# ferreiraluisa/implementation-phd-lab-vision

Measured on AMD Instinct MI355X. Metric: H36M frames/sec ResNet-50 feature extraction, higher is better.
Workload: dtype bf16; 1 GPU; ResNet-50[:-1] bf16 forward, batch 256 x 224x224x3 fp32 NCHW frames per GPU (BASELINE configs[1]), seeded synthetic weights, (N,2048) fp32 features; batch_per_gpu=256, micro_batch=0, lanes=2, lanes_requested=2, lanes_mode=2 lanes (1.081 x one lane), input=f32, parallelism=frames sharded over 1 rank(s)

## Files before the change

### implementation_phd_lab_vision_amd/_lib.py

```python
from __future__ import annotations

import ctypes as C
import os
import subprocess
from pathlib import Path
from typing import Optional

PKG_DIR = Path(__file__).resolve().parent
LIB_PATH = Path(os.environ.get("R50_LIB", str(PKG_DIR / "libr50hip.so")))
CSRC = PKG_DIR / "csrc"

HIPCC_FLAGS = ["--offload-arch=gfx950", "-O3", "-std=c++17", "-fPIC", "-shared", "-ffp-contract=off"]


class R50Error(RuntimeError):
    pass


class TensorDesc(C.Structure):
    _fields_ = [("name", C.c_char_p), ("data", C.POINTER(C.c_float)), ("numel", C.c_int64)]


def _source_digest() -> str:
    import hashlib
# ... 82 lines not shown
                                            C.c_void_p, C.c_int, C.c_void_p]),
    "r50_op_transpose16": (C.c_int, [C.c_void_p, C.c_int, C.c_int, C.c_void_p, C.c_int, C.c_void_p]),
    "r50_op_mask_scale": (C.c_int, [C.c_void_p, C.c_void_p, C.c_float, C.c_int64, C.c_int, C.c_void_p]),
    "r50_op_relu_bwd": (C.c_int, [C.c_void_p, C.c_void_p, C.c_float, C.c_int64, C.c_int, C.c_void_p]),
    "r50_op_colsum": (C.c_int, [C.c_void_p, C.c_int64, C.c_int, C.c_int, C.c_float, C.c_void_p, C.c_int, C.c_int, C.c_void_p]),
    "r50_op_colsum_f32": (C.c_int, [C.c_void_p, C.c_int64, C.c_int, C.c_float, C.c_void_p, C.c_int, C.c_void_p]),
    "r50_op_grad_accum": (C.c_int, [C.c_void_p, C.c_float, C.c_void_p, C.c_int64, C.c_int, C.c_int, C.c_void_p]),
    "r50_op_mse_loss_grad": (C.c_int, [C.c_void_p, C.c_void_p, C.c_int64, C.c_float, C.c_void_p, C.c_void_p, C.c_void_p]),
    "r50_op_gn_relu_causal3_bwd": (C.c_int, [C.c_void_p, C.c_void_p, C.c_int, C.c_int, C.c_int, C.c_int, C.c_void_p, C.c_void_p,
                                             C.c_float, C.c_void_p, C.c_void_p, C.c_void_p, C.c_void_p, C.c_int, C.c_void_p]),
    "r50_op_check_finite": (C.c_int, [C.c_void_p, C.c_int64, C.c_void_p, C.c_void_p]),
    "r50_op_check_overflow16": (C.c_int, [C.c_void_p, C.c_int64, C.c_void_p, C.c_int, C.c_void_p]),
    "r50_op_adamw": (C.c_int, [C.c_void_p, C.c_void_p, C.c_void_p, C.c_void_p, C.c_void_p, C.c_int64, C.c_float, C.c_float, C.c_float,
                               C.c_float, C.c_float, C.c_int, C.c_void_p, C.c_int, C.c_void_p]),
    "r50_op_avgpool": (C.c_int, [C.c_void_p, C.c_int, C.c_int, C.c_int, C.c_void_p, C.c_void_p]),
    "r50_op_pose_metrics": (C.c_int, [C.c_void_p, C.c_void_p, C.c_int64, C.c_int, C.c_void_p, C.c_void_p]),
    "r50_op_horizon_metrics": (C.c_int, [C.c_void_p, C.c_void_p, C.c_int, C.c_int, C.c_int, C.c_int, C.c_int, C.c_void_p, C.c_void_p]),
    "r50_op_pose_protocols": (C.c_int, [C.c_void_p, C.c_void_p, C.c_void_p, C.c_int, C.c_int, C.c_int, C.c_int, C.c_int, C.c_int,
                                        C.c_int, C.c_void_p, C.c_void_p]),
    "r50_op_pose_detail_metrics": (C.c_int, [C.c_void_p, C.c_void_p, C.c_void_p, C.c_int, C.c_int, C.c_int, C.c_int, C.c_int, C.c_int,
                                             C.c_int, C.c_int, C.c_double, C.c_void_p, C.c_void_p]),
    "r50_op_future_pose_loss_grad": (C.c_int, [C.c_void_p, C.c_void_p, C.c_int, C.c_int, C.c_int, C.c_float, C.c_void_p, C.c_void_p,
                                               C.c_void_p]),
    "r50_op_ar_latent_grad": (C.c_int, [C.c_void_p, C.c_void_p, C.c_void_p, C.c_int, C.c_int, C.c_int, C.c_float, C.c_float, C.c_void_p,
                                        C.c_void_p, C.c_void_p, C.c_int, C.c_void_p]),
    "r50_op_colsum_split": (C.c_int, [C.c_void_p, C.c_int64, C.c_int, C.c_int, C.c_float, C.c_void_p, C.c_void_p, C.c_int, C.c_int,
                                      C.c_void_p]),
    "r50_op_joint_pose_loss_grad": (C.c_int, [C.c_void_p, C.c_void_p, C.c_int, C.c_int, C.c_int, C.c_float, C.c_float, C.c_void_p,
                                              C.c_void_p, C.c_void_p]),
    "r50_op_gn_relu_causal3_tm_bwd": (C.c_int, [C.c_void_p, C.c_void_p, C.c_int, C.c_int, C.c_int, C.c_int, C.c_int, C.c_void_p, C.c_void_p,
# ... 38 lines not shown
```

### implementation_phd_lab_vision_amd/csrc/kernels.h

```cpp
#pragma once
#include <hip/hip_runtime.h>
#include <stdint.h>
#include <type_traits>

typedef __attribute__((ext_vector_type(8))) __bf16 bf16x8;
typedef __attribute__((ext_vector_type(4))) float f32x4;
typedef __attribute__((ext_vector_type(4))) unsigned int u32x4;
typedef __attribute__((ext_vector_type(2))) unsigned int u32x2;

#define GLOBAL_AS __attribute__((address_space(1)))
#define LDS_AS __attribute__((address_space(3)))

__device__ __forceinline__ float bf16_bits_to_f32(unsigned int hi16) { return __uint_as_float(hi16 << 16); }

__device__ __forceinline__ unsigned int pack_bf16x2(float lo, float hi) {
    typedef __attribute__((ext_vector_type(2))) __bf16 bf16x2;
    typedef __attribute__((ext_vector_type(2))) float f32x2;
    f32x2 v = {lo, hi};
    bf16x2 b = __builtin_convertvector(v, bf16x2);
    return __builtin_bit_cast(unsigned int, b);
}

typedef __attribute__((ext_vector_type(8))) _Float16 f16x8;
typedef __attribute__((ext_vector_type(2))) _Float16 f16x2;
// ... 67 lines not shown
    int n_blocks;
    int x_back;
    unsigned x_records;
    unsigned w_bytes;
    unsigned y_bytes;
    FastDiv div_howo, div_wo, div_ctiles;
    int x_cstride;
    int x_wrap;
    int y_cstride;
    int et;
    float oscale, rscale;
    float q_inv;
    const __bf16* x2;
    int H2, W2, stride2, x2_cstride, cc1;
    unsigned x2_records;
#if defined(R50_STAMP)
    unsigned long long* dbg;
#endif
};

#if defined(R50_STAMP)
#define R50_STAMP_DECL unsigned long long st_prev = __builtin_readcyclecounter(), st_sum[8] = {0, 0, 0, 0, 0, 0, 0, 0}; const unsigned long long st_rt0 = __builtin_amdgcn_s_memrealtime();
#define R50_MARK(i) { __builtin_amdgcn_sched_barrier(0); const unsigned long long st_now = __builtin_readcyclecounter(); st_sum[i] += st_now - st_prev; st_prev = st_now; __builtin_amdgcn_sched_barrier(0); }
#define R50_STAMP_FLUSH(nw) st_sum[7] = __builtin_amdgcn_s_memrealtime() - st_rt0;    \
    if (a.dbg && (threadIdx.x & 63) == 0) { _Pragma("unroll") for (int q = 0; q < 8; ++q) \
        a.dbg[((size_t)blockIdx.x * (nw) + (threadIdx.x >> 6)) * 8 + q] = st_sum[q]; }
#else
#define R50_STAMP_DECL
#define R50_MARK(i)
#define R50_STAMP_FLUSH(nw)
// ... 20 lines not shown
        constexpr int MID = (LO + HI) / 2;
        if (n <= MID) wait_vmcnt_range<LO, MID>(n);
        else wait_vmcnt_range<MID + 1, HI>(n);
    }
}
__device__ __forceinline__ void wait_vmcnt(int n) { wait_vmcnt_range<0, 63>(n < 0 ? 0 : (n > 63 ? 63 : n)); }

__device__ __forceinline__ unsigned relu_bf16x2(unsigned v) {
    typedef __attribute__((ext_vector_type(2))) short s16x2;
    const s16x2 z = {0, 0};
    return __builtin_bit_cast(unsigned, __builtin_elementwise_max(__builtin_bit_cast(s16x2, v), z));
}

constexpr unsigned kOobOffset = 0x80000000u;

template <int ET, int BC, int BP, int WC, int WP, int NSTAGE, bool SPLIT = false>
__global__ __launch_bounds__(WC * WP * 64) void igemm_bf16_kernel(const ConvArgs a) {
#if defined(__HIP_DEVICE_COMPILE__)
    constexpr int NT = WC * WP * 64;
    constexpr int MR = BC / WC / 16;
    constexpr int NR = BP / WP / 16;
    static_assert(MR >= 2 && (MR % 2) == 0, "wave needs >= 32 couts");
    static_assert(NSTAGE == 2 || NSTAGE == 3, "2 or 3 LDS stages");
    constexpr int RPP = NT / 8;
    static_assert(BC % RPP == 0 && BP % (16 * WP) == 0, "cout rows fill whole staging passes; pixels come in 16-blocks per wave");
    constexpr int WROWS = BC / RPP;
    constexpr int XROWS = (BP + RPP - 1) / RPP;
    constexpr int BP_PAD = XROWS * RPP;
    constexpr int PASS_BYTES = NT * 16;
    constexpr int STAGE_BYTES = (BC + BP_PAD) * 128;
    constexpr int LOADS_PER_STAGE = WROWS + XROWS;
    constexpr int D = NSTAGE - 1;

    extern __shared__ __attribute__((aligned(16))) char smem[];

    const int tid = threadIdx.x;
    const int lane = tid & 63;
    const int wave = __builtin_amdgcn_readfirstlane(tid >> 6);
    const int wave_c = wave / WP, wave_p = wave % WP;
    const int fr = lane & 15, fq = lane >> 4;
    const int srow = tid >> 3;
    const int slot = tid & 7;
    const int lchunk = slot ^ (srow & 7);

    const int grid = gridDim.x;
    const int first = xcd_remap(blockIdx.x, grid);
    const int my_tiles = (a.n_blocks - first + grid - 1) / grid;
    const int total = my_tiles * a.nk;

    const __amdgpu_buffer_rsrc_t rsrc_w =
        __builtin_amdgcn_make_buffer_rsrc(const_cast<__bf16*>(a.w), 0, a.w_bytes, 0x00020000);
    const __amdgpu_buffer_rsrc_t rsrc_x = __builtin_amdgcn_make_buffer_rsrc(
        const_cast<char*>(reinterpret_cast<const char*>(a.x) - a.x_back), 0, a.x_records, 0x00020000);
    const __amdgpu_buffer_rsrc_t rsrc_y = __builtin_amdgcn_make_buffer_rsrc(a.y, 0, a.y_bytes, 0x00020000);
    const __amdgpu_buffer_rsrc_t rsrc_r =
        __builtin_amdgcn_make_buffer_rsrc(const_cast<__bf16*>(a.res), 0, a.res ? a.y_bytes : 0u, 0x00020000);

    unsigned x_voff[XROWS], x_mask[XROWS], w_voff[WROWS];
    auto decode_tile = [&](int tile) {
        const int pt = (int)fast_div((unsigned)tile, a.div_ctiles);
        const int ct = tile - pt * a.n_ctiles;
        const int c0 = ct * BC, p0 = pt * BP;
#pragma unroll
        for (int i = 0; i < XROWS; ++i) {
            const int m = p0 + i * RPP + srow;
            unsigned mask = 0u, voff = kOobOffset;
            if ((BP_PAD == BP || i * RPP + srow < BP) && m < a.M) {
                const int n = (int)fast_div((unsigned)m, a.div_howo);
                const int r = m - n * a.HoWo;
                const int ho = (int)fast_div((unsigned)r, a.div_wo);
                const int wo = r - ho * a.Wo;
                const int hc = ho * a.stride, wc = wo * a.stride;
                voff = (unsigned)(((n * a.H + hc) * a.W + wc) * a.x_cstride + lchunk * 8) * 2u;
                if (a.ks == 1) {
                    mask = 1u;
                } else {
                    const unsigned hm = (hc >= a.pad ? 1u : 0u) | 2u | (hc - a.pad + 2 < a.H ? 4u : 0u);
                    const unsigned wm = (wc >= a.pad ? 1u : 0u) | 2u | (wc - a.pad + 2 < a.W ? 4u : 0u);
                    mask = ((hm & 1u) ? wm : 0u) | ((hm & 2u) ? (wm << 3) : 0u) | ((hm & 4u) ? (wm << 6) : 0u);
                }
            }
            x_voff[i] = voff;
// ... 40 lines not shown
        }
    };

    f32x4 acc[MR][NR];
    constexpr bool BIG = (MR * NR > 16);
    constexpr bool LEAN = (NT >= 1024);
    constexpr bool PREFETCH_RES = !SPLIT && !BIG && !LEAN;
    u32x4 res_reg[PREFETCH_RES ? MR / 2 : 1][PREFETCH_RES ? NR : 1];
    const bool has_res = (a.res != nullptr);
    const int fphys0 = (fq ^ (fr & 7)) << 4;
    const int w_frag = (wave_c * MR * 16 + fr) * 128;
    const int x_frag = BC * 128 + (wave_p * NR * 16 + fr) * 128;
    const int cout_lane = wave_c * MR * 16 + 8 * fq;
    const int pix_lane = wave_p * NR * 16 + fr;
    int c_tile = first, c_k = 0, c_buf = 0;
    unsigned y_voff = 0u;
    const unsigned y_rowstep = (unsigned)(16 * a.y_cstride * 2);

    auto tile_begin = [&]() {
        const int pt = (int)fast_div((unsigned)c_tile, a.div_ctiles);
        const int c0 = (c_tile - pt * a.n_ctiles) * BC, p0 = pt * BP;
        y_voff = (unsigned)((p0 + pix_lane) * a.y_cstride + c0 + cout_lane) * 2u;
#pragma unroll
        for (int t = 0; t < MR / 2; ++t) {
            const f32x4 b_lo = *reinterpret_cast<const f32x4*>(a.bias + c0 + cout_lane + 32 * t);
            const f32x4 b_hi = *reinterpret_cast<const f32x4*>(a.bias + c0 + cout_lane + 32 * t + 4);
#pragma unroll
            for (int j = 0; j < NR; ++j) {
                acc[2 * t][j] = b_lo;
                acc[2 * t + 1][j] = b_hi;
                if constexpr (PREFETCH_RES) if (has_res)
                    res_reg[t][j] = __builtin_amdgcn_raw_buffer_load_b128(rsrc_r, y_voff + j * y_rowstep + 64 * t, 0, 0);
            }
        }
    };
    auto compute = [&]() {
        const char* sbase = smem + c_buf * STAGE_BYTES;
// ... 25 lines not shown
                wf[kk][m] = *reinterpret_cast<const bf16x8*>(sbase + w_frag + m * 2048 + ph);
        }
#pragma unroll
        for (int kk = 0; kk < 2; ++kk)
#pragma unroll
            for (int m = 0; m < MR; ++m)
#pragma unroll
                for (int j = 0; j < NR; ++j)
                    acc[m][j] = mfma_e<ET>(wf[kk][m], xf[kk][j], acc[m][j]);
        if constexpr (BIG) {
            __builtin_amdgcn_sched_group_barrier(0x100, 2 * (MR + NR), 0);
            __builtin_amdgcn_sched_group_barrier(0x008, 2 * MR * NR, 0);
        }
        }
    };
    auto epilogue = [&]() {
#pragma unroll
        for (int t = 0; t < MR / 2; ++t) {
#pragma unroll
            for (int j = 0; j < NR; ++j) {
                f32x4 lo = acc[2 * t][j], hi = acc[2 * t + 1][j];
                const unsigned voff = y_voff + j * y_rowstep + 64 * t;
                if constexpr (!SPLIT) {
                    if (has_res) {
                        u32x4 r;
                        if constexpr (PREFETCH_RES) r = res_reg[t][j];
                        else r = __builtin_amdgcn_raw_buffer_load_b128(rsrc_r, voff, 0, 0);
                        lo[0] += unpack_lo_e<ET>(r[0]); lo[1] += unpack_hi_e<ET>(r[0]);
                        lo[2] += unpack_lo_e<ET>(r[1]); lo[3] += unpack_hi_e<ET>(r[1]);
                        hi[0] += unpack_lo_e<ET>(r[2]); hi[1] += unpack_hi_e<ET>(r[2]);
                        hi[2] += unpack_lo_e<ET>(r[3]); hi[3] += unpack_hi_e<ET>(r[3]);
// ... 32 lines not shown
                }
            }
        }
    };

#pragma unroll
    for (int s = 0; s < D; ++s)
        if (s < total) stage_issue();
    for (int g = 0; g < total; ++g) {
        if (NSTAGE == 3 && g + 1 < total) {
            asm volatile("s_waitcnt vmcnt(%0)" ::"n"(LOADS_PER_STAGE) : "memory");
        } else {
            asm volatile("s_waitcnt vmcnt(0)" ::: "memory");
        }
        __builtin_amdgcn_s_barrier();
        if (c_k == 0) tile_begin();
        if (g + D < total) stage_issue();
        compute();
        c_buf = (c_buf == NSTAGE - 1) ? 0 : c_buf + 1;
        if (++c_k == a.nk) {
            epilogue();
            c_k = 0;
            c_tile += grid;
        }
    }
#else
    (void)a;
#endif
}

template <int ET, int BC, int BP, int CWC, int CWP, int NLOAD, int NSTAGE>
__global__ __launch_bounds__((CWC * CWP + NLOAD) * 64) void igemm_ws_kernel(const ConvArgs a) {
#if defined(__HIP_DEVICE_COMPILE__)
    constexpr int NCONS = CWC * CWP;
    constexpr int MR = BC / CWC / 16;
    constexpr int NR = BP / CWP / 16;
    static_assert(MR >= 2 && (MR % 2) == 0, "consumer wave needs >= 32 couts");
    static_assert(BP % (16 * CWP) == 0, "pixels come in 16-blocks per consumer wave");
// ... 4795 lines not shown
```

### implementation_phd_lab_vision_amd/csrc/r50_abi.hip

```cpp
#include "kernels.h"
#include "../../include/r50.h"

#include <atomic>
#include <cmath>
#include <cstdlib>
#include <cstdio>
#include <cstring>
#include <map>
#include <string>
#include <vector>

namespace {

thread_local std::string g_err;

struct Prof {
    const char* name;
    int64_t launches = 0;
    double ms = 0, flops = 0, bytes = 0;
};
enum ProfClass { PC_IGEMM = 0, PC_STEM_CONV, PC_MAXPOOL, PC_AVGPOOL, PC_STEM_PACK, PC_TAIL, PC_TAIL3, PC_BLOCK2, PC_CATCHAIN, PC_COUNT };
const char* kProfNames[PC_COUNT] = {"igemm", "conv1", "maxpool", "avgpool", "stem_pack", "bneck_tail", "bneck_tail3", "bneck_block2", "bneck_catchain"};

struct EvRec {
// ... 31 lines not shown
    std::vector<float> fp8_scales;
    float cat_acc_scale[4] = {0.f, 0.f, 0.f, 0.f};
    int fuse_ds_cat = 1;
    __bf16* cat_w[4] = {nullptr, nullptr, nullptr, nullptr};
    float* cat_bias[4] = {nullptr, nullptr, nullptr, nullptr};
    int fuse_tail = 1;
    int fuse_fp8_handover = 1;
    int fuse_tail3 = 1;
    __bf16* catchain_wp = nullptr;
    int fuse_tail3_last = 1;
    int fuse_cat_chain = 1;
    int sub_out = 1;
    __bf16* tail3_wp[8] = {nullptr, nullptr, nullptr, nullptr, nullptr, nullptr, nullptr, nullptr};
    int fuse_block1 = 3;
    int fuse_block2 = 1;
    int inplace_out = 0;
    int n_streams = 1;
    hipStream_t side[4] = {nullptr, nullptr, nullptr, nullptr};
    hipEvent_t ev_fork = nullptr, ev_join[4] = {nullptr, nullptr, nullptr, nullptr};
    bool loaded = false;
    r50_handle* owner = nullptr;
    int sharers = 0;
    bool zombie = false;
    std::string err;
    std::vector<ConvLayer> convs;
    char* stem_w = nullptr;
    char* stem_xp = nullptr;
    float* u8_table = nullptr;
    __bf16* buf[5] = {nullptr, nullptr, nullptr, nullptr, nullptr};
    size_t buf_bytes = 0;
// ... 217 lines not shown
            int dev = 0;
            hipDeviceProp_t prop;
            if (hipGetDevice(&dev) != hipSuccess || hipGetDeviceProperties(&prop, dev) != hipSuccess) return hipErrorInvalidDevice;
            g_num_cus = cu_budget(prop.multiProcessorCount);
        }
        static int per_cu = 0;
        if (per_cu == 0) {
            int n = 0;
            if (hipOccupancyMaxActiveBlocksPerMultiprocessor(&n, kern, WC * WP * 64, lds) != hipSuccess || n < 1) n = 1;
            per_cu = n;
        }
        if (grid > g_num_cus * per_cu) grid = g_num_cus * per_cu;
    }
    hipLaunchKernelGGL(kern, dim3(grid), dim3(WC * WP * 64), lds, s, a);
    return hipGetLastError();
}

struct TunedTile { int h, cin, cout, ks, stride, res, tile; };
constexpr TunedTile kTuned[] = {
    {56, 64, 64, 1, 1, 0, 73},    {56, 64, 64, 3, 1, 0, 2},     {56, 64, 256, 1, 1, 1, 72},   {56, 64, 256, 1, 1, 0, 38},
    {56, 256, 64, 1, 1, 0, 73},    {56, 256, 128, 1, 1, 0, 40},  {56, 128, 128, 3, 2, 0, 65},   {28, 128, 512, 1, 1, 1, 72},
    {56, 256, 512, 1, 2, 0, 42},  {28, 512, 128, 1, 1, 0, 65},   {28, 128, 128, 3, 1, 0, 72},  {28, 512, 256, 1, 1, 0, 72},
    {28, 256, 256, 3, 2, 0, 44},  {14, 256, 1024, 1, 1, 1, 72}, {28, 512, 1024, 1, 2, 0, 72}, {14, 1024, 256, 1, 1, 0, 44},
    {14, 256, 256, 3, 1, 0, 68},  {14, 1024, 512, 1, 1, 0, 72}, {14, 512, 512, 3, 2, 0, 68},  {7, 512, 2048, 1, 1, 1, 43},
    {14, 1024, 2048, 1, 2, 0, 43}, {7, 2048, 512, 1, 1, 0, 72}, {7, 512, 512, 3, 1, 0, 68},
};

constexpr int kWsBit = 64;

template <int ET, int BC, int BP, int CWC, int CWP, int NLOAD, int NSTAGE>
// ... 282 lines not shown
    a.cin_chunks = kmul * (cin / 64); a.nk = ks * ks * a.cin_chunks; a.Ktot = ks * ks * kmul * cin;
    a.n_ctiles = 0; a.n_blocks = 0;
    const long long x_bytes = (long long)n * h * w * a.x_cstride * 2;
    a.x_back = (pad * w + pad) * a.x_cstride * 2;
    if (x_bytes + a.x_back >= (1ll << 31) || (long long)cout * a.Ktot * 2 >= (1ll << 31) || M * a.y_cstride * 2 >= (1ll << 31))
        return R50_ERR_INVALID;
    a.x_records = (unsigned)(x_bytes + a.x_back);
    a.w_bytes = (unsigned)((long long)cout * a.Ktot * 2);
    a.y_bytes = (unsigned)(M * a.y_cstride * 2);
    a.div_howo = make_fast_div((unsigned)a.HoWo);
    a.div_wo = make_fast_div((unsigned)a.Wo);
    a.div_ctiles = FastDiv{0u, 0u};
    a.et = 0;
    a.oscale = 1.0f; a.rscale = 1.0f; a.q_inv = 0.0f;
    a.x2 = nullptr; a.H2 = 0; a.W2 = 0; a.stride2 = 1; a.x2_cstride = 0; a.cc1 = 1 << 30; a.x2_records = 0u;
#if defined(R50_STAMP)
    a.dbg = nullptr;
#endif
    return R50_OK;
}

void prof_begin(r50_handle* h, hipStream_t s, EvRec& r, int cls, double flops, double bytes, int layer = -1) {
    if (!h || !h->profile) return;
    r.layer = layer;
    auto get = [&]() {
        hipEvent_t e;
        if (!h->ev_free.empty()) { e = h->ev_free.back(); h->ev_free.pop_back(); }
        else (void)hipEventCreate(&e);
        return e;
    };
// ... 510 lines not shown
    }
    if (hit("stem", buf[0], 112, 112, 64)) return R50_OK;

    prof_begin(h, s, r, PC_MAXPOOL, 0, (double)n * (112.0 * 112 + 56.0 * 56) * 64 * 2 * cmul);
    e = split ? launch_maxpool_split(buf[0], buf[1], n, 112, 112, 64, s) : launch_maxpool(buf[0], buf[1], n, 112, 112, 64, s, et);
    prof_end(h, s, r);
    if (e != hipSuccess) return fail(h, R50_ERR_HIP, std::string("maxpool: ") + hipGetErrorString(e));
after_pool:
    if (hit("pool", buf[1], 56, 56, 64)) return R50_OK;

    int cur = 1, hh = 56, ww = 56;
    int pre_t1 = stem_c1 ? 2 : -1;
    bool layer1_out_fp8 = false;
    bool cur_sub = false;
    size_t li = 1;
    for (int si = 0; si < 4; ++si) {
        const int blocks = kStages[si][1];
        if (si == 1 && h->precision == R50_PREC_FP8) {
            if (tap) return fail(h, R50_ERR_INVALID, "fp8 mode: activations beyond layer1 are e4m3 tensors, taps stop at layer1.2");
            return run_fp8_part(h, buf, cur, n, out, s, layer1_out_fp8);
        }
        for (int b = 0; b < blocks; ++b) {
            int fr[4], nf = 0;
            if (pre_t1 >= 0) fr[nf++] = pre_t1;
            for (int i = 0; i < 5; ++i)
                if (i != cur && i != pre_t1) fr[nf++] = i;
            const bool have_t1 = (pre_t1 >= 0);
            pre_t1 = -1;
            if (cur_sub && !(si == 1 && b == 0)) return fail(h, R50_ERR_STATE, "internal: a sub-sampled block output reached a block that reads the full tensor");
            const std::string p = "layer" + std::to_string(si + 1) + "." + std::to_string(b);
// ... 160 lines not shown
                pre_t1 = fr[0];
            } else if (cat_ds) {
                rc = run_conv_cat(h, si, c3, *cdp, buf[fr[1]], buf[cur], n, h2, w2, hh, ww, outb, s);
                if (rc) return rc;
                h3 = h2; w3 = w2;
            } else if (si == 2 && b == blocks - 1 && b < 8 && h->tail3_wp[b] && h->fuse_tail3 && h->fuse_tail3_last && h->fuse_tail && !split && !tap && h->tile_override == 0 &&
                       (h->precision == R50_PREC_BF16 || h->precision == R50_PREC_FP16) && c3.ks == 1 && c3.cin == 256 && c3.cout == 1024 && idn == buf[cur]) {
                const long long m = (long long)n * h2 * w2;
                EvRec rt{};
                prof_begin(h, s, rt, PC_TAIL3, 2.0 * m * (double)c3.cout * c3.cin, 2.0 * (m * ((double)c3.cin + 2.0 * c3.cout) + (double)c3.cout * c3.cin),
                           (int)(&c3 - &h->convs[0]));
                e = launch_bneck_tail3(buf[fr[1]], m, h->tail3_wp[b], c3.bias, idn, outb, nullptr, nullptr, s, et, 0, true);
                prof_end(h, s, rt);
                if (e != hipSuccess) return fail(h, R50_ERR_HIP, "bneck_tail3 (no next conv1) launch (" + c3.conv_key + "): " + hipGetErrorString(e));
                h3 = h2; w3 = w2;
            } else {
                const bool handover = (h->precision == R50_PREC_FP8 && h->fuse_fp8_handover && si == 0 && b == blocks - 1 && !tap &&
                                       (int)h->fp8_scales.size() == R50_FP8_NUM_SCALES);
                rc = run_conv(h, c3, buf[fr[1]], n, h2, w2, idn, outb, 1, s, &h3, &w3, handover ? 1.0f / h->fp8_scales[0] : 0.f,
                              handover ? &layer1_out_fp8 : nullptr);
                if (rc) return rc;
            }
            if (!inplace) cur = fr[3];
            hh = h3; ww = w3;
            if (hit(p, buf[cur], hh, ww, c3.cout)) return R50_OK;
            li += (b == 0) ? 4 : 3;
        }
    }
    if (tap) return fail(h, R50_ERR_INVALID, std::string("unknown layer name: ") + tap);
    prof_begin(h, s, r, PC_AVGPOOL, 0, (double)n * (hh * ww * 2048.0 * 2 + 2048.0 * 4));
    e = split ? launch_avgpool_split(buf[cur], out, n, hh * ww, 2048, s) : launch_avgpool(buf[cur], out, n, hh * ww, 2048, s, et);
    prof_end(h, s, r);
    if (e != hipSuccess) return fail(h, R50_ERR_HIP, std::string("avgpool: ") + hipGetErrorString(e));
    return R50_OK;
}

void free_weights(r50_handle* h) {
    const bool own = (h->owner == nullptr);
    for (auto& L : h->convs) {
        if (own && L.w) (void)hipFree(L.w);
        if (own && L.bias) (void)hipFree(L.bias);
        if (L.bias_scaled) (void)hipFree(L.bias_scaled);
        L.w = nullptr; L.bias = nullptr; L.bias_scaled = nullptr;
    }
// ... 385 lines not shown
    else if (k == "fuse_cat_chain") h->fuse_cat_chain = value ? 1 : 0;
    else if (k == "sub_out") h->sub_out = value ? 1 : 0;
    else if (k == "fuse_tail3_last") h->fuse_tail3_last = value ? 1 : 0;
    else if (k == "tail3_bp") { if (value < 0 || value > 112) return fail(h, R50_ERR_INVALID, "tail3_bp must be 0 .. 112"); g_tail3_bp = (int)value; }
    else if (k == "fuse_fp8_handover") h->fuse_fp8_handover = value ? 1 : 0;
    else if (k == "fuse_stem_c1") h->fuse_stem_c1 = value ? 1 : 0;
    else if (k == "fuse_ds_cat") h->fuse_ds_cat = value ? 1 : 0;
    else if (k == "stem_strip") {
        if (!(value == 0 || (value > 0 && 28 % value == 0))) return fail(h, R50_ERR_INVALID, "stem_strip must be 0 or a divisor of 28");
        g_stem_strip = (int)value;
    }
    else if (k == "overlap_ds") h->overlap_ds = value ? 1 : 0;
    else if (k == "streams") { if (value < 1 || value > 4) return fail(h, R50_ERR_INVALID, "streams must be in [1,4]"); h->n_streams = (int)value; }
    else if (k == "inplace_out") h->inplace_out = value ? 1 : 0;
    else if (k == "fuse_block2") h->fuse_block2 = value ? 1 : 0;
    else if (k == "fuse_block1") { if (value < 0 || value > 3) return fail(h, R50_ERR_INVALID, "fuse_block1 must be 0 .. 3"); h->fuse_block1 = (int)value; }
    else if (k == "use_g8") { if (value < 0 || value > 3) return fail(h, R50_ERR_INVALID, "use_g8 must be 0 .. 3"); g_use_g8 = (int)value; }
    else if (k == "use_s2") g_use_s2 = (int)value;
    else if (k == "cu_cap") { if (value < 0 || value > 4096) return fail(h, R50_ERR_INVALID, "cu_cap must be in [0,4096]"); g_cu_cap = (int)value; g_num_cus = 0; }
    else return fail(h, R50_ERR_INVALID, "r50_set_option: unknown key " + k);
    return R50_OK;
}

int r50_get_option(r50_handle* h, const char* key, int64_t* value) {
    if (!h || !key || !value) return fail(h, R50_ERR_INVALID, "r50_get_option: null argument");
    const std::string k(key);
    if (k == "micro_batch") *value = h->micro_batch;
    else if (k == "profile") *value = h->profile;
    else if (k == "tile") *value = h->tile_override;
    else if (k == "streams") *value = h->n_streams;
    else if (k == "cu_cap") *value = g_cu_cap;
    else if (k == "inplace_out") *value = h->inplace_out;
    else if (k == "fuse_block2") *value = h->fuse_block2;
    else if (k == "fuse_block1") *value = h->fuse_block1;
    else if (k == "fused_stem") *value = h->fused_stem;
    else if (k == "fuse_tail") *value = h->fuse_tail;
    else if (k == "fuse_tail3") *value = h->fuse_tail3;
    else if (k == "tail3_bp") *value = g_tail3_bp;
    else if (k == "use_g8") *value = g_use_g8;
    else if (k == "fuse_cat_chain") *value = h->fuse_cat_chain;
    else if (k == "sub_out") *value = h->sub_out;
    else if (k == "fuse_tail3_last") *value = h->fuse_tail3_last;
    else if (k == "fuse_fp8_handover") *value = h->fuse_fp8_handover;
    else if (k == "fuse_stem_c1") *value = h->fuse_stem_c1;
    else if (k == "fuse_ds_cat") *value = h->fuse_ds_cat;
    else if (k == "stem_strip") *value = g_stem_strip;
    else if (k == "overlap_ds") *value = h->overlap_ds;
    else if (k == "max_batch") *value = h->max_batch;
// ... 639 lines not shown
    hipStream_t s = (hipStream_t)stream;
    HIP_TRY(nullptr, hipMemcpyAsync(scratch, pk.data(), STEM_W_BYTES, hipMemcpyHostToDevice, s));
    HIP_TRY(nullptr, hipStreamSynchronize(s));
    char* xp = (char*)scratch + STEM_W_BYTES;
    HIP_TRY(nullptr, launch_stem_pack(x, xp, n, s));
    HIP_TRY(nullptr, launch_stem_conv(xp, scratch, bias_dev, y, n, s));
    return R50_OK;
}

int r50_op_maxpool(const void* x, int n, int h, int w, int c, void* y, void* stream) {
    if (!x || !y || n < 1 || h < 1 || w < 1 || c < 8 || c % 8) return fail(nullptr, R50_ERR_INVALID, "r50_op_maxpool: invalid arguments");
    HIP_TRY(nullptr, launch_maxpool(x, y, n, h, w, c, (hipStream_t)stream));
    return R50_OK;
}

int r50_op_avgpool(const void* x, int n, int hw, int c, float* y, void* stream) {
    if (!x || !y || n < 1 || hw < 1 || c < 8 || c % 8) return fail(nullptr, R50_ERR_INVALID, "r50_op_avgpool: invalid arguments");
    HIP_TRY(nullptr, launch_avgpool(x, y, n, hw, c, (hipStream_t)stream));
    return R50_OK;
}

}
```

### implementation_phd_lab_vision_amd/ops.py

```python
from __future__ import annotations

from typing import Optional

import torch

from . import _lib

TILE_AUTO = 0
TILE_128x128 = 1
TILE_64x128 = 2
TILE_64x256 = 3
TILE_128x64 = 5
TILE_256x128_P3 = 6
TILE_128x256_P3 = 7
TILE_128x128_P3 = 8
TILE_256x256 = 9
TILE_256x256_B = 10
TILE_256x208 = 11
TILE_256x224 = 12
WS = 64
TILE_XRES = 81
TILE_S2 = 82
TILE_G8 = 83
TILE_G8_224 = 84
# ... 244 lines not shown
    _lib.check(rc, None, "r50_op_stem")
    return y


def maxpool_bf16(x: torch.Tensor) -> torch.Tensor:
    _need(x, torch.bfloat16, "x")
    n, h, w, c = x.shape
    y = torch.empty((n, (h - 1) // 2 + 1, (w - 1) // 2 + 1, c), dtype=torch.bfloat16, device=x.device)
    with torch.cuda.device(x.device):
        rc = _lib.load_library().r50_op_maxpool(x.data_ptr(), n, h, w, c, y.data_ptr(), _stream(x))
    _lib.check(rc, None, "r50_op_maxpool")
    return y


def avgpool_bf16(x: torch.Tensor) -> torch.Tensor:
    _need(x, torch.bfloat16, "x")
    n, h, w, c = x.shape
    y = torch.empty((n, c), dtype=torch.float32, device=x.device)
    with torch.cuda.device(x.device):
        rc = _lib.load_library().r50_op_avgpool(x.data_ptr(), n, h * w, c, y.data_ptr(), _stream(x))
    _lib.check(rc, None, "r50_op_avgpool")
    return y
```

### include/r50.h

```cpp
#ifndef R50_H_
#define R50_H_

#include <stdint.h>

#ifdef __cplusplus
extern "C" {
#endif

typedef struct r50_handle r50_handle;

typedef enum r50_status {
    R50_OK = 0,
    R50_ERR_INVALID = -1,
    R50_ERR_HIP = -2,
    R50_ERR_STATE = -3,
    R50_ERR_NOMEM = -4
} r50_status;

typedef enum r50_precision {
    R50_PREC_BF16 = 1,
    R50_PREC_FP32X = 2,
    R50_PREC_BF16W2 = 3,
    R50_PREC_FP16 = 4,
    R50_PREC_FP8 = 5
// ... 132 lines not shown
                                float* out4, void* stream);

int r50_op_gn_relu_causal3_tm_bwd(const void* dr, const void* x, int b, int t, int t0, int c, int groups, const float* gamma,
                                  const float* beta, float eps, const void* add, void* dx, float* dgamma_part, float* dbeta_part, int et,
                                  void* stream);
int r50_op_rollout_pose_loss_grad(const float* pred, const float* gt, int b, int k, int t_gt, int i0, int joints, float loss_scale,
                                  float* dy, float* loss2, void* stream);
int r50_op_rollout_latent_grad(const void* fut, const void* phi, int b, int k, int t_phi, int i0, int d, float lambda, float loss_scale,
                               float* dfut, float* loss_lat, float* row_part, int et, void* stream);

int r50_op_geo_pose_loss_grad(const float* y, const float* gt3d, const float* gt2d, const float* K, int b, int t, int s0, int joints,
                              const int* edges_host, int n_edges, float lambda_2d, float lambda_vel, float lambda_bone, float eps,
                              float term_scale, float loss_scale, float* dy, double* part, float* out8, void* stream);

int r50_op_avgpool(const void* x_nhwc_bf16, int n, int hw, int c, float* y_f32, void* stream);

#ifdef __cplusplus
}
#endif
#endif
```

Baseline: 105,300 frames/s.

## Fuse final conv1x1 residual/ReLU epilogue with global average pooling

Adds a POOL variant of the implicit-GEMM kernel for the last bottleneck conv3 (7x7, 512->2048). Each wave takes four whole images, adds the residual, applies ReLU, stages the bf16 result in an LDS patch and column-sums it, so the pooled fp32 features are written directly. This skips writing the 7x7x2048 activation and the separate avgpool kernel launch and re-read. In exchange the kernel uses a 208-pixel tile stepping by 196, which wastes some MMA work, and needs extra LDS that may lower occupancy. It also adds an fp16 avgpool entry point and a Python wrapper.

```diff
diff --git a/implementation_phd_lab_vision_amd/_lib.py b/implementation_phd_lab_vision_amd/_lib.py
--- a/implementation_phd_lab_vision_amd/_lib.py
+++ b/implementation_phd_lab_vision_amd/_lib.py
@@ -120,6 +120,9 @@
     "r50_op_adamw": (C.c_int, [C.c_void_p, C.c_void_p, C.c_void_p, C.c_void_p, C.c_void_p, C.c_int64, C.c_float, C.c_float, C.c_float,
                                C.c_float, C.c_float, C.c_int, C.c_void_p, C.c_int, C.c_void_p]),
     "r50_op_avgpool": (C.c_int, [C.c_void_p, C.c_int, C.c_int, C.c_int, C.c_void_p, C.c_void_p]),
+    "r50_op_avgpool_f16": (C.c_int, [C.c_void_p, C.c_int, C.c_int, C.c_int, C.c_void_p, C.c_void_p]),
+    "r50_op_conv1x1_pool": (C.c_int, [C.c_void_p, C.c_int, C.c_int, C.c_int, C.c_void_p, C.c_void_p, C.c_void_p, C.c_int, C.c_void_p,
+                                      C.c_int, C.c_void_p]),
     "r50_op_pose_metrics": (C.c_int, [C.c_void_p, C.c_void_p, C.c_int64, C.c_int, C.c_void_p, C.c_void_p]),
     "r50_op_horizon_metrics": (C.c_int, [C.c_void_p, C.c_void_p, C.c_int, C.c_int, C.c_int, C.c_int, C.c_int, C.c_void_p, C.c_void_p]),
     "r50_op_pose_protocols": (C.c_int, [C.c_void_p, C.c_void_p, C.c_void_p, C.c_int, C.c_int, C.c_int, C.c_int, C.c_int, C.c_int,
diff --git a/implementation_phd_lab_vision_amd/csrc/kernels.h b/implementation_phd_lab_vision_amd/csrc/kernels.h
--- a/implementation_phd_lab_vision_amd/csrc/kernels.h
+++ b/implementation_phd_lab_vision_amd/csrc/kernels.h
@@ -105,6 +105,8 @@
     const __bf16* x2;
     int H2, W2, stride2, x2_cstride, cc1;
     unsigned x2_records;
+    float* pool_out;
+    float inv_hw;
 #if defined(R50_STAMP)
     unsigned long long* dbg;
 #endif
@@ -155,7 +157,9 @@
 
 constexpr unsigned kOobOffset = 0x80000000u;
 
-template <int ET, int BC, int BP, int WC, int WP, int NSTAGE, bool SPLIT = false>
+constexpr int POOL_HW = 49, POOL_IMGS = 4, POOL_PIX = POOL_HW * POOL_IMGS, POOL_WAVE_BYTES = POOL_HW * 64;
+
+template <int ET, int BC, int BP, int WC, int WP, int NSTAGE, bool SPLIT = false, bool POOL = false>
 __global__ __launch_bounds__(WC * WP * 64) void igemm_bf16_kernel(const ConvArgs a) {
 #if defined(__HIP_DEVICE_COMPILE__)
     constexpr int NT = WC * WP * 64;
@@ -172,6 +176,8 @@
     constexpr int STAGE_BYTES = (BC + BP_PAD) * 128;
     constexpr int LOADS_PER_STAGE = WROWS + XROWS;
     constexpr int D = NSTAGE - 1;
+    constexpr int PSTEP = POOL ? POOL_PIX : BP;
+    static_assert(!POOL || (!SPLIT && WP == 1 && MR == 2 && BP >= POOL_PIX), "pooling epilogue: a wave holds 32 couts x four whole 7x7 images");
 
     extern __shared__ __attribute__((aligned(16))) char smem[];
 
@@ -201,12 +207,12 @@
     auto decode_tile = [&](int tile) {
         const int pt = (int)fast_div((unsigned)tile, a.div_ctiles);
         const int ct = tile - pt * a.n_ctiles;
-        const int c0 = ct * BC, p0 = pt * BP;
+        const int c0 = ct * BC, p0 = pt * PSTEP;
 #pragma unroll
         for (int i = 0; i < XROWS; ++i) {
             const int m = p0 + i * RPP + srow;
             unsigned mask = 0u, voff = kOobOffset;
-            if ((BP_PAD == BP || i * RPP + srow < BP) && m < a.M) {
+            if ((BP_PAD == PSTEP || i * RPP + srow < PSTEP) && m < a.M) {
                 const int n = (int)fast_div((unsigned)m, a.div_howo);
                 const int r = m - n * a.HoWo;
                 const int ho = (int)fast_div((unsigned)r, a.div_wo);
@@ -277,13 +283,15 @@
     const int cout_lane = wave_c * MR * 16 + 8 * fq;
     const int pix_lane = wave_p * NR * 16 + fr;
     int c_tile = first, c_k = 0, c_buf = 0;
+    int c_img0 = 0, c_cout0 = 0;
     unsigned y_voff = 0u;
     const unsigned y_rowstep = (unsigned)(16 * a.y_cstride * 2);
 
     auto tile_begin = [&]() {
         const int pt = (int)fast_div((unsigned)c_tile, a.div_ctiles);
-        const int c0 = (c_tile - pt * a.n_ctiles) * BC, p0 = pt * BP;
+        const int c0 = (c_tile - pt * a.n_ctiles) * BC, p0 = pt * PSTEP;
         y_voff = (unsigned)((p0 + pix_lane) * a.y_cstride + c0 + cout_lane) * 2u;
+        if constexpr (POOL) { c_img0 = pt * POOL_IMGS; c_cout0 = c0; }
 #pragma unroll
         for (int t = 0; t < MR / 2; ++t) {
             const f32x4 b_lo = *reinterpret_cast<const f32x4*>(a.bias + c0 + cout_lane + 32 * t);
@@ -339,7 +347,71 @@
         }
         }
     };
+    auto pool_epilogue = [&]() {
+        char* const patch = smem + NSTAGE * STAGE_BYTES + wave * POOL_WAVE_BYTES;
+        u32x4 pk[NR];
+        u32x4 rr[NR];
+        __builtin_amdgcn_sched_barrier(0);
+        if (has_res) {
+#pragma unroll
+            for (int j = 0; j < NR; ++j) {
+                const unsigned voff = (16 * j + 15 < POOL_PIX || fr + 16 * j < POOL_PIX) ? y_voff + j * y_rowstep : kOobOffset;
+                rr[j] = __builtin_amdgcn_raw_buffer_load_b128(rsrc_r, voff, 0, 0);
+            }
+        }
+#pragma unroll
+        for (int j = 0; j < NR; ++j) {
+            __builtin_amdgcn_sched_barrier(0);
+            f32x4 lo = acc[0][j], hi = acc[1][j];
+            if (has_res) {
+                const u32x4 r = rr[j];
+                lo[0] += unpack_lo_e<ET>(r[0]); lo[1] += unpack_hi_e<ET>(r[0]);
+                lo[2] += unpack_lo_e<ET>(r[1]); lo[3] += unpack_hi_e<ET>(r[1]);
+                hi[0] += unpack_lo_e<ET>(r[2]); hi[1] += unpack_hi_e<ET>(r[2]);
+                hi[2] += unpack_lo_e<ET>(r[3]); hi[3] += unpack_hi_e<ET>(r[3]);
+            }
+            pk[j] = (u32x4){pack2_e<ET>(lo[0], lo[1]), pack2_e<ET>(lo[2], lo[3]), pack2_e<ET>(hi[0], hi[1]), pack2_e<ET>(hi[2], hi[3])};
+            if (a.relu) {
+#pragma unroll
+                for (int e = 0; e < 4; ++e) pk[j][e] = relu_bf16x2(pk[j][e]);
+            }
+        }
+        __builtin_amdgcn_sched_barrier(0);
+        char* const wbase = patch + fr * 64 + fq * 16 - 3 * 64;
+        auto wave_sync = [&]() {
+            __builtin_amdgcn_fence(__ATOMIC_RELEASE, "wavefront");
+            __builtin_amdgcn_wave_barrier();
+            __builtin_amdgcn_fence(__ATOMIC_ACQUIRE, "wavefront");
+        };
+#pragma unroll
+        for (int img = 0; img < POOL_IMGS; ++img) {
+#pragma unroll
+            for (int j = (POOL_HW * img) / 16; j <= (POOL_HW * img + POOL_HW - 1) / 16; ++j) {
+                const int ql = fr + 16 * j - POOL_HW * img;
+                if (ql >= 0 && ql < POOL_HW) *reinterpret_cast<u32x4*>(wbase + (16 * j - POOL_HW * img + 3) * 64) = pk[j];
+            }
+            wave_sync();
+            float s_lo = 0.f, s_hi = 0.f;
+            const char* col = patch + fr * 4;
+            unsigned v[POOL_HW];
+#pragma unroll
+            for (int r = 0; r < POOL_HW; ++r) v[r] = *reinterpret_cast<const unsigned*>(col + r * 64);
+#pragma unroll
+            for (int r = 0; r < POOL_HW; ++r) {
+                if (r % 7 == 0) __builtin_amdgcn_sched_barrier(0);
+                s_lo += unpack_lo_e<ET>(v[r]);
+                s_hi += unpack_hi_e<ET>(v[r]);
+            }
+            wave_sync();
+            if (fq == 0 && c_img0 + img < a.N) {
+                typedef __attribute__((ext_vector_type(2))) float f32x2;
+                float* o = a.pool_out + (size_t)(c_img0 + img) * a.Cout + c_cout0 + wave_c * 32 + 2 * fr;
+                *reinterpret_cast<f32x2*>(o) = (f32x2){s_lo * a.inv_hw, s_hi * a.inv_hw};
+            }
+        }
+    };
     auto epilogue = [&]() {
+        if constexpr (POOL) { pool_epilogue(); return; }
 #pragma unroll
         for (int t = 0; t < MR / 2; ++t) {
 #pragma unroll
@@ -402,7 +474,7 @@
             asm volatile("s_waitcnt vmcnt(0)" ::: "memory");
         }
         __builtin_amdgcn_s_barrier();
-        if (c_k == 0) tile_begin();
+        if (c_k == 0 && (!POOL || g == 0)) tile_begin();
         if (g + D < total) stage_issue();
         compute();
         c_buf = (c_buf == NSTAGE - 1) ? 0 : c_buf + 1;
@@ -410,6 +482,7 @@
             epilogue();
             c_k = 0;
             c_tile += grid;
+            if constexpr (POOL) tile_begin();
         }
     }
 #else
diff --git a/implementation_phd_lab_vision_amd/csrc/r50_abi.hip b/implementation_phd_lab_vision_amd/csrc/r50_abi.hip
--- a/implementation_phd_lab_vision_amd/csrc/r50_abi.hip
+++ b/implementation_phd_lab_vision_amd/csrc/r50_abi.hip
@@ -69,6 +69,7 @@
     __bf16* tail3_wp[8] = {nullptr, nullptr, nullptr, nullptr, nullptr, nullptr, nullptr, nullptr};
     int fuse_block1 = 3;
     int fuse_block2 = 1;
+    int fuse_pool = 1;
     int inplace_out = 0;
     int n_streams = 1;
     hipStream_t side[4] = {nullptr, nullptr, nullptr, nullptr};
@@ -316,6 +317,36 @@
     }
     hipLaunchKernelGGL(kern, dim3(grid), dim3(WC * WP * 64), lds, s, a);
     return hipGetLastError();
+}
+
+bool is_pool_shape(const ConvArgs& a) {
+    return a.ks == 1 && a.stride == 1 && a.pad == 0 && a.HoWo == POOL_HW && a.Cout % 256 == 0 && a.x2 == nullptr && a.x_cstride == a.Cin &&
+           a.y_cstride == a.Cout && a.x_wrap >= (1 << 30) && a.q_inv == 0.f && (a.et == 0 || a.et == 1);
+}
+template <int ET>
+hipError_t launch_igemm_pool_t(ConvArgs a, hipStream_t s) {
+    constexpr int BC = 256, BP = 208, NT = 512;
+    constexpr size_t lds = 2 * (size_t)(BC + (BP + NT / 8 - 1) / (NT / 8) * (NT / 8)) * 128 + (NT / 64) * (size_t)POOL_WAVE_BYTES;
+    static_assert(lds <= 163840, "LDS budget");
+    auto kern = igemm_bf16_kernel<ET, BC, BP, 8, 1, 2, false, true>;
+    hipError_t e = hipFuncSetAttribute(reinterpret_cast<const void*>(kern), hipFuncAttributeMaxDynamicSharedMemorySize, (int)lds);
+    if (e != hipSuccess) return e;
+    if (g_num_cus == 0) {
+        int dev = 0;
+        hipDeviceProp_t prop;
+        if (hipGetDevice(&dev) != hipSuccess || hipGetDeviceProperties(&prop, dev) != hipSuccess) return hipErrorInvalidDevice;
+        g_num_cus = cu_budget(prop.multiProcessorCount);
+    }
+    a.n_ctiles = a.Cout / BC;
+    a.n_blocks = a.n_ctiles * ((a.N + POOL_IMGS - 1) / POOL_IMGS);
+    a.div_ctiles = make_fast_div((unsigned)a.n_ctiles);
+    const int grid = a.n_blocks < g_num_cus ? a.n_blocks : g_num_cus;
+    hipLaunchKernelGGL(kern, dim3(grid), dim3(NT), lds, s, a);
+    return hipGetLastError();
+}
+hipError_t launch_igemm_pool(const ConvArgs& a, hipStream_t s) {
+    if (!a.pool_out || !is_pool_shape(a)) return hipErrorInvalidValue;
+    return a.et == 1 ? launch_igemm_pool_t<1>(a, s) : launch_igemm_pool_t<0>(a, s);
 }
 
 struct TunedTile { int h, cin, cout, ks, stride, res, tile; };
@@ -628,6 +659,7 @@
     a.et = 0;
     a.oscale = 1.0f; a.rscale = 1.0f; a.q_inv = 0.0f;
     a.x2 = nullptr; a.H2 = 0; a.W2 = 0; a.stride2 = 1; a.x2_cstride = 0; a.cc1 = 1 << 30; a.x2_records = 0u;
+    a.pool_out = nullptr; a.inv_hw = 0.f;
 #if defined(R50_STAMP)
     a.dbg = nullptr;
 #endif
@@ -1168,6 +1200,7 @@
     bool layer1_out_fp8 = false;
     bool cur_sub = false;
     size_t li = 1;
+    bool pooled = false;
     for (int si = 0; si < 4; ++si) {
         const int blocks = kStages[si][1];
         if (si == 1 && h->precision == R50_PREC_FP8) {
@@ -1358,6 +1391,20 @@
                 prof_end(h, s, rt);
                 if (e != hipSuccess) return fail(h, R50_ERR_HIP, "bneck_tail3 (no next conv1) launch (" + c3.conv_key + "): " + hipGetErrorString(e));
                 h3 = h2; w3 = w2;
+            } else if (h->fuse_pool && si == 3 && b == blocks - 1 && (h->precision == R50_PREC_BF16 || h->precision == R50_PREC_FP16) && !split && !tap &&
+                       h->tile_override == 0 && h2 == 7 && w2 == 7 && c3.ks == 1 && c3.stride == 1 && c3.cin == 512 && c3.cout == 2048 && idn == buf[cur]) {
+                ConvArgs a;
+                rc = fill_conv_args(a, buf[fr[1]], n, h2, w2, c3.cin, c3.w, c3.bias, idn, outb, c3.cout, 1, 1, 0, 1);
+                if (rc) return fail(h, rc, "conv args invalid for " + c3.conv_key);
+                a.et = et; a.y = nullptr; a.pool_out = out; a.inv_hw = 1.0f / (float)(h2 * w2);
+                EvRec rt{};
+                prof_begin(h, s, rt, PC_IGEMM, 2.0 * a.M * (double)c3.cout * c3.cin,
+                           2.0 * ((double)a.M * c3.cin + (double)a.M * c3.cout + (double)c3.cout * c3.cin) + (double)n * c3.cout * 4.0, (int)(&c3 - &h->convs[0]));
+                e = launch_igemm_pool(a, s);
+                prof_end(h, s, rt);
+                if (e != hipSuccess) return fail(h, R50_ERR_HIP, "igemm + pool launch (" + c3.conv_key + "): " + hipGetErrorString(e));
+                h3 = h2; w3 = w2;
+                pooled = true;
             } else {
                 const bool handover = (h->precision == R50_PREC_FP8 && h->fuse_fp8_handover && si == 0 && b == blocks - 1 && !tap &&
                                        (int)h->fp8_scales.size() == R50_FP8_NUM_SCALES);
@@ -1372,6 +1419,7 @@
         }
     }
     if (tap) return fail(h, R50_ERR_INVALID, std::string("unknown layer name: ") + tap);
+    if (pooled) return R50_OK;
     prof_begin(h, s, r, PC_AVGPOOL, 0, (double)n * (hh * ww * 2048.0 * 2 + 2048.0 * 4));
     e = split ? launch_avgpool_split(buf[cur], out, n, hh * ww, 2048, s) : launch_avgpool(buf[cur], out, n, hh * ww, 2048, s, et);
     prof_end(h, s, r);
@@ -1787,6 +1835,7 @@
     else if (k == "streams") { if (value < 1 || value > 4) return fail(h, R50_ERR_INVALID, "streams must be in [1,4]"); h->n_streams = (int)value; }
     else if (k == "inplace_out") h->inplace_out = value ? 1 : 0;
     else if (k == "fuse_block2") h->fuse_block2 = value ? 1 : 0;
+    else if (k == "fuse_pool") h->fuse_pool = value ? 1 : 0;
     else if (k == "fuse_block1") { if (value < 0 || value > 3) return fail(h, R50_ERR_INVALID, "fuse_block1 must be 0 .. 3"); h->fuse_block1 = (int)value; }
     else if (k == "use_g8") { if (value < 0 || value > 3) return fail(h, R50_ERR_INVALID, "use_g8 must be 0 .. 3"); g_use_g8 = (int)value; }
     else if (k == "use_s2") g_use_s2 = (int)value;
@@ -1805,6 +1854,7 @@
     else if (k == "cu_cap") *value = g_cu_cap;
     else if (k == "inplace_out") *value = h->inplace_out;
     else if (k == "fuse_block2") *value = h->fuse_block2;
+    else if (k == "fuse_pool") *value = h->fuse_pool;
     else if (k == "fuse_block1") *value = h->fuse_block1;
     else if (k == "fused_stem") *value = h->fused_stem;
     else if (k == "fuse_tail") *value = h->fuse_tail;
@@ -2474,6 +2524,25 @@
     return R50_OK;
 }
 
+int r50_op_conv1x1_pool(const void* x, int n, int hw, int cin, const void* wt, const float* bias, const void* res, int cout, float* out,
+                        int et, void* stream) {
+    if (hw != POOL_HW || !out || (et != 0 && et != 1)) return fail(nullptr, R50_ERR_INVALID, "r50_op_conv1x1_pool: hw must be 49 (7x7), et 0 or 1");
+    ConvArgs a;
+    int rc = fill_conv_args(a, x, n, 7, 7, cin, wt, bias, res, out, cout, 1, 1, 0, 1);
+    if (rc || cout % 256) return fail(nullptr, R50_ERR_INVALID, "r50_op_conv1x1_pool: invalid arguments (cin % 64, cout % 256)");
+    a.et = et; a.y = nullptr; a.pool_out = out; a.inv_hw = 1.0f / (float)hw;
+    hipError_t e = launch_igemm_pool(a, (hipStream_t)stream);
+    if (e != hipSuccess) return fail(nullptr, e == hipErrorInvalidValue ? R50_ERR_INVALID : R50_ERR_HIP,
+                                     std::string("r50_op_conv1x1_pool: ") + hipGetErrorString(e));
+    return R50_OK;
+}
+
+int r50_op_avgpool_f16(const void* x, int n, int hw, int c, float* y, void* stream) {
+    if (!x || !y || n < 1 || hw < 1 || c < 8 || c % 8) return fail(nullptr, R50_ERR_INVALID, "r50_op_avgpool_f16: invalid arguments");
+    HIP_TRY(nullptr, launch_avgpool(x, y, n, hw, c, (hipStream_t)stream, 1));
+    return R50_OK;
+}
+
 int r50_op_avgpool(const void* x, int n, int hw, int c, float* y, void* stream) {
     if (!x || !y || n < 1 || hw < 1 || c < 8 || c % 8) return fail(nullptr, R50_ERR_INVALID, "r50_op_avgpool: invalid arguments");
     HIP_TRY(nullptr, launch_avgpool(x, y, n, hw, c, (hipStream_t)stream));
diff --git a/implementation_phd_lab_vision_amd/ops.py b/implementation_phd_lab_vision_amd/ops.py
--- a/implementation_phd_lab_vision_amd/ops.py
+++ b/implementation_phd_lab_vision_amd/ops.py
@@ -282,10 +282,37 @@
 
 
 def avgpool_bf16(x: torch.Tensor) -> torch.Tensor:
-    _need(x, torch.bfloat16, "x")
+    et = x.dtype
+    if et not in (torch.bfloat16, torch.float16):
+        raise ValueError("avgpool_bf16: x must be bf16 or fp16")
+    _need(x, et, "x")
     n, h, w, c = x.shape
     y = torch.empty((n, c), dtype=torch.float32, device=x.device)
-    with torch.cuda.device(x.device):
-        rc = _lib.load_library().r50_op_avgpool(x.data_ptr(), n, h * w, c, y.data_ptr(), _stream(x))
+    lib = _lib.load_library()
+    with torch.cuda.device(x.device):
+        fn = lib.r50_op_avgpool if et == torch.bfloat16 else lib.r50_op_avgpool_f16
+        rc = fn(x.data_ptr(), n, h * w, c, y.data_ptr(), _stream(x))
     _lib.check(rc, None, "r50_op_avgpool")
     return y
+
+
+def conv1x1_pool(x: torch.Tensor, w: torch.Tensor, bias: torch.Tensor, residual: Optional[torch.Tensor] = None) -> torch.Tensor:
+    et = x.dtype
+    if et not in (torch.bfloat16, torch.float16):
+        raise ValueError("conv1x1_pool: x must be bf16 or fp16")
+    _need(x, et, "x"); _need(w, et, "w"); _need(bias, torch.float32, "bias")
+    n, h, wd, cin = x.shape
+    cout = w.shape[0]
+    if w.numel() != cout * cin or bias.numel() != cout:
+        raise ValueError("conv1x1_pool: inconsistent shapes")
+    if residual is not None:
+        _need(residual, et, "residual")
+        if tuple(residual.shape) != (n, h, wd, cout):
+            raise ValueError("conv1x1_pool: residual shape mismatch")
+    y = torch.empty((n, cout), dtype=torch.float32, device=x.device)
+    with torch.cuda.device(x.device):
+        rc = _lib.load_library().r50_op_conv1x1_pool(x.data_ptr(), n, h * wd, cin, w.data_ptr(), bias.data_ptr(),
+                                                     residual.data_ptr() if residual is not None else None, cout, y.data_ptr(),
+                                                     0 if et == torch.bfloat16 else 1, _stream(x))
+    _lib.check(rc, None, "r50_op_conv1x1_pool")
+    return y
diff --git a/include/r50.h b/include/r50.h
--- a/include/r50.h
+++ b/include/r50.h
@@ -170,6 +170,10 @@
                               float term_scale, float loss_scale, float* dy, double* part, float* out8, void* stream);
 
 int r50_op_avgpool(const void* x_nhwc_bf16, int n, int hw, int c, float* y_f32, void* stream);
+int r50_op_avgpool_f16(const void* x_nhwc_f16, int n, int hw, int c, float* y_f32, void* stream);
+
+int r50_op_conv1x1_pool(const void* x_nhwc, int n, int hw, int cin, const void* w_oi, const float* bias_f32, const void* residual_nhwc,
+                        int cout, float* out_f32, int et, void* stream);
 
 #ifdef __cplusplus
 }
```

Result: no change. 105,300 frames/s, median of 2 (+0.0%).
